# kv13arm/mujoco_rl_manipulate_unknown_objects

Hardware: NVIDIA B200
Metric: env-steps/sec (acorn_env, 4096 envs/GPU) (higher is better)
Workload: dtype f32

## Files before the change

mujoco_rl_manipulate_unknown_objects_b200/csrc/sim_kernels.cuh:

```cuda
#pragma once
#include <cuda_runtime.h>
#include <stdint.h>

#include "model.h"

namespace grs {

constexpr int MAXCON = 12;
constexpr int MAXEFC = MAXCON * 4 + 7;
constexpr unsigned FULL = 0xffffffffu;
constexpr float MINVAL = 1e-15f;

struct __align__(16) WS {
  float qpos[16], qvel[16], ctrl[8], warm[16];
  float xpos[MAXB][3], xquat[MAXB][4], xmat[MAXB][9];
  float xanchor[MAXJ][3], xaxis[MAXJ][3];
  float gpos[MAXG][3], gmat[MAXG][9];
  float com[MAXB][3];
  float cdof[16][6];
  float M[NV * NV];
  int ncon, nefc, nlim, overflow, coupled, padi[3];
  float c_dist[MAXCON], c_pos[MAXCON][3], c_frame[MAXCON][9], c_mu[MAXCON], c_fric[MAXCON][3];
  int c_g1[MAXCON], c_g2[MAXCON], c_pair[MAXCON];
  float fsmooth[16], asmooth[16], qacc[16], Ma[16], grad[16], search[16], Mv[16], fcon[16], bias[16];
  float e_D[MAXEFC], e_aref[MAXEFC], e_jar[MAXEFC], e_Jv[MAXEFC], e_force[MAXEFC], e_act[MAXEFC];
  float hc[MAXCON][16];
  int istate[32];
  float tgt[8], init_q[8], out[40];
  float sup[5][9];
  float cho[16];
  float sep[MAXPAIR][3];
  float gapb[MAXPAIR];
  float disp[MAXG];
  union {
    struct {
      float xipos[MAXB][3], ximat[MAXB][9], cinert[MAXB][10], crb[MAXB][10], cdofdot[16][6], cvel[MAXB][6], cfrc[MAXB][6];
      float L[NV * NV];
    } dyn;
    struct {
      float J[MAXEFC][NV];
      float H[NV * NV];
    } con;
  } u;
};

struct StepStats { int iters_total, max_iters, ncon_max; };

__device__ __forceinline__ float warp_sum(float v) {
#pragma unroll
  for (int o = 16; o > 0; o >>= 1) v += __shfl_xor_sync(FULL, v, o);
  return v;
}
__device__ __forceinline__ float dot3(const float* a, const float* b) { return a[0] * b[0] + a[1] * b[1] + a[2] * b[2]; }
__device__ __forceinline__ void cross3(float* r, const float* a, const float* b) {
  float x = a[1] * b[2] - a[2] * b[1], y = a[2] * b[0] - a[0] * b[2], z = a[0] * b[1] - a[1] * b[0];
  r[0] = x; r[1] = y; r[2] = z;
}
__device__ __forceinline__ float normalize3(float* a) {
  float n = sqrtf(dot3(a, a));
  if (n < MINVAL) { a[0] = 1; a[1] = 0; a[2] = 0; return n; }
  float inv = 1.0f / n;
  a[0] *= inv; a[1] *= inv; a[2] *= inv;
  return n;
}
__device__ __forceinline__ void quat_mul(float* r, const float* a, const float* b) {
  float t0 = a[0] * b[0] - a[1] * b[1] - a[2] * b[2] - a[3] * b[3];
  float t1 = a[0] * b[1] + a[1] * b[0] + a[2] * b[3] - a[3] * b[2];
  float t2 = a[0] * b[2] - a[1] * b[3] + a[2] * b[0] + a[3] * b[1];
  float t3 = a[0] * b[3] + a[1] * b[2] - a[2] * b[1] + a[3] * b[0];
  r[0] = t0; r[1] = t1; r[2] = t2; r[3] = t3;
}
__device__ __forceinline__ void quat_normalize(float* q) {
  float n = sqrtf(q[0] * q[0] + q[1] * q[1] + q[2] * q[2] + q[3] * q[3]);
  if (n < MINVAL) { q[0] = 1; q[1] = q[2] = q[3] = 0; return; }
  float inv = 1.0f / n;
  q[0] *= inv; q[1] *= inv; q[2] *= inv; q[3] *= inv;
}
__device__ __forceinline__ void quat2mat(float* R, const float* q) {
  float w = q[0], x = q[1], y = q[2], z = q[3];
  R[0] = w * w + x * x - y * y - z * z; R[1] = 2 * (x * y - w * z); R[2] = 2 * (x * z + w * y);
  R[3] = 2 * (x * y + w * z); R[4] = w * w - x * x + y * y - z * z; R[5] = 2 * (y * z - w * x);
  R[6] = 2 * (x * z - w * y); R[7] = 2 * (y * z + w * x); R[8] = w * w - x * x - y * y + z * z;
}
__device__ __forceinline__ void mulmat3vec(float* r, const float* R, const float* v) {
  float x = R[0] * v[0] + R[1] * v[1] + R[2] * v[2], y = R[3] * v[0] + R[4] * v[1] + R[5] * v[2], z = R[6] * v[0] + R[7] * v[1] + R[8] * v[2];
  r[0] = x; r[1] = y; r[2] = z;
}
__device__ __forceinline__ void mulmat3Tvec(float* r, const float* R, const float* v) {
  float x = R[0] * v[0] + R[3] * v[1] + R[6] * v[2], y = R[1] * v[0] + R[4] * v[1] + R[7] * v[2], z = R[2] * v[0] + R[5] * v[1] + R[8] * v[2];
  r[0] = x; r[1] = y; r[2] = z;
}
__device__ __forceinline__ void rot_vec_quat(float* r, const float* v, const float* q) {
  float R[9];
  quat2mat(R, q);
  mulmat3vec(r, R, v);
}
__device__ __forceinline__ void mul_inert_vec(float* r, const float* c, const float* v) {
  float t[3];
  r[0] = c[0] * v[0] + c[3] * v[1] + c[4] * v[2];
  r[1] = c[3] * v[0] + c[1] * v[1] + c[5] * v[2];
  r[2] = c[4] * v[0] + c[5] * v[1] + c[2] * v[2];
  cross3(t, c + 6, v + 3);
  r[0] += t[0]; r[1] += t[1]; r[2] += t[2];
  cross3(t, c + 6, v);
  r[3] = c[9] * v[3] - t[0]; r[4] = c[9] * v[4] - t[1]; r[5] = c[9] * v[5] - t[2];
}
__device__ __forceinline__ float dot6(const float* a, const float* b) { return a[0] * b[0] + a[1] * b[1] + a[2] * b[2] + a[3] * b[3] + a[4] * b[4] + a[5] * b[5]; }
__device__ __forceinline__ void cross_motion(float* r, const float* v, const float* mv) {
  float t[3];
  cross3(r, v, mv);
  cross3(r + 3, v, mv + 3);
  cross3(t, v + 3, mv);
  r[3] += t[0]; r[4] += t[1]; r[5] += t[2];
}
__device__ __forceinline__ void cross_force(float* r, const float* v, const float* f) {
  float t[3];
  cross3(r, v, f);
  cross3(t, v + 3, f + 3);
  r[0] += t[0]; r[1] += t[1]; r[2] += t[2];
  cross3(r + 3, v, f + 3);
}

template <bool BLOCKS>
__device__ __noinline__ float chol_factor_solve(float* A, float* tmp, float b, int lane) {
  constexpr int NB = BLOCKS ? 7 : NV;
  const bool is_row = lane < NV;
  const bool is_rhs = BLOCKS ? (lane == 13 || lane == 14) : (lane == NV);
  const int base = BLOCKS ? (((lane >= 7 && lane < NV) || lane == 14) ? 7 : 0) : 0;
  const int nb = BLOCKS ? (base ? 6 : 7) : NV;
  const int lr = is_rhs ? NB : lane - base;
  if (is_row) tmp[lane] = b;
  __syncwarp();
  float a[NB];
#pragma unroll
  for (int k = 0; k < NB; k++) {
    a[k] = 0.0f;
    if (k < nb) {
      if (is_row && k <= lr) a[k] = A[lane * NV + base + k];
      else if (is_rhs) a[k] = tmp[base + k];
    }
  }
#pragma unroll
  for (int j = 0; j < NB; j++) {
    if (is_row && lr >= j) A[lane * NV + base + j] = a[j];
    __syncwarp();
    const int cj = base + (j < nb ? j : 0);
    const float djj = A[cj * NV + cj];
    float rs = rsqrtf(fmaxf(djj, 1e-30f));
    rs = rs * (1.5f - 0.5f * djj * rs * rs);
    const float t = a[j] * rs * rs;
    a[j] *= rs;
#pragma unroll
    for (int k = j + 1; k < NB; k++) {
      const int rk = base + (k < nb ? k : 0);
      a[k] -= t * A[rk * NV + cj];
    }
  }
  __syncwarp();
  if (is_row) {
#pragma unroll
    for (int k = 0; k < NB; k++)
      if (k <= lr) A[lane * NV + base + k] = a[k];
  }
  if (is_rhs) {
#pragma unroll
    for (int k = 0; k < NB; k++)
      if (k < nb) tmp[base + k] = a[k];
  }
  __syncwarp();
  float y = is_row ? tmp[lane] : 0.0f;
#pragma unroll
  for (int j = NB - 1; j >= 0; j--) {
    const bool valid = j < nb;
    const int gj = base + (valid ? j : 0);
    const float ljj = A[gj * NV + gj];
    if (is_row && valid && lr == j) tmp[gj] = __fdividef(y, ljj);
    __syncwarp();
    const float xj = tmp[gj];
    if (is_row && valid) {
      if (lr == j) y = xj;
      else if (lr < j) y -= A[gj * NV + lane] * xj;
    }
  }
  __syncwarp();
  return y;
}

__device__ __noinline__ void kinematics(const DevModel& m, WS& w, int lane) {
  if (lane == 0) {
    for (int j = 0; j < m.njnt; j++)
      if (m.jnt_type[j] == JNT_FREE) quat_normalize(w.qpos + m.jnt_qposadr[j] + 3);
    w.xpos[0][0] = w.xpos[0][1] = w.xpos[0][2] = 0;
    w.xquat[0][0] = 1; w.xquat[0][1] = w.xquat[0][2] = w.xquat[0][3] = 0;
    quat2mat(w.xmat[0], w.xquat[0]);
  }
  __syncwarp();
  for (int lv = 1; lv < m.nlevel; lv++) {
    int idx = m.level_start[lv] + lane;
    if (idx < m.level_start[lv + 1]) {
      int b = m.level_body[idx], pid = m.body_parent[b];
      int jadr = m.body_jntadr[b], jnum = m.body_jntnum[b];
      float pos[3], quat[4];
      if (jnum == 1 && m.jnt_type[jadr] == JNT_FREE) {
        int qa = m.jnt_qposadr[jadr];
        for (int k = 0; k < 3; k++) pos[k] = w.qpos[qa + k];
        for (int k = 0; k < 4; k++) quat[k] = w.qpos[qa + 3 + k];
        for (int k = 0; k < 3; k++) { w.xanchor[jadr][k] = pos[k]; w.xaxis[jadr][k] = 0; }
      } else {
        float t[3];
        mulmat3vec(t, w.xmat[pid], m.body_pos[b]);
        for (int k = 0; k < 3; k++) pos[k] = w.xpos[pid][k] + t[k];
        quat_mul(quat, w.xquat[pid], m.body_quat[b]);
        for (int kj = 0; kj < jnum; kj++) {
          int j = jadr + kj;
          float anchor[3], axis[3];
          rot_vec_quat(t, m.jnt_pos[j], quat);
          for (int k = 0; k < 3; k++) anchor[k] = pos[k] + t[k];
          rot_vec_quat(axis, m.jnt_axis[j], quat);
          float q = w.qpos[m.jnt_qposadr[j]] - m.jnt_qpos0[j];
          if (m.jnt_type[j] == JNT_SLIDE) {
            for (int k = 0; k < 3; k++) pos[k] += axis[k] * q;
          } else {
            float s, c, ql[4];
            sincosf(0.5f * q, &s, &c);
            ql[0] = c; ql[1] = m.jnt_axis[j][0] * s; ql[2] = m.jnt_axis[j][1] * s; ql[3] = m.jnt_axis[j][2] * s;
            quat_mul(quat, quat, ql);
            rot_vec_quat(t, m.jnt_pos[j], quat);
            for (int k = 0; k < 3; k++) pos[k] = anchor[k] - t[k];
          }
          for (int k = 0; k < 3; k++) { w.xanchor[j][k] = anchor[k]; w.xaxis[j][k] = axis[k]; }
        }
      }
      quat_normalize(quat);
      for (int k = 0; k < 3; k++) w.xpos[b][k] = pos[k];
      for (int k = 0; k < 4; k++) w.xquat[b][k] = quat[k];
      quat2mat(w.xmat[b], quat);
    }
    __syncwarp();
  }
  if (lane < m.ngeom) {
    int g = lane, b = m.geom_body[g];
    float t[3], q[4], R[9];
    mulmat3vec(t, w.xmat[b], m.geom_pos[g]);
    quat_mul(q, w.xquat[b], m.geom_quat[g]);
    quat_normalize(q);
    quat2mat(R, q);
    float d2 = 0, r2 = 0;
    for (int k = 0; k < 3; k++) { const float np_ = w.xpos[b][k] + t[k], d = np_ - w.gpos[g][k]; d2 += d * d; w.gpos[g][k] = np_; }
    for (int k = 0; k < 9; k++) { const float d = R[k] - w.gmat[g][k]; r2 += d * d; w.gmat[g][k] = R[k]; }
    w.disp[g] = sqrtf(d2) + m.geom_rbound[g] * sqrtf(r2);
  }
  __syncwarp();
}

__device__ __noinline__ void com_pos_crb(const DevModel& m, WS& w, int lane) {
  const int nb = m.nbody;
  if (lane < nb) {
    int b = lane;
    float t[3], qi[4];
    mulmat3vec(t, w.xmat[b], m.body_ipos[b]);
    for (int k = 0; k < 3; k++) w.u.dyn.xipos[b][k] = w.xpos[b][k] + t[k];
    quat_mul(qi, w.xquat[b], m.body_iquat[b]);
    quat2mat(w.u.dyn.ximat[b], qi);
  }
  __syncwarp();
  if (lane < nb) {
    int r = m.body_root[lane];
    unsigned mask = m.body_subtree_mask[r];
    float s[3] = {0, 0, 0}, ms = 0;
    for (int b = 1; b < nb; b++)
      if ((mask >> b) & 1u) {
        float mb = m.body_mass[b];
        ms += mb;
        for (int k = 0; k < 3; k++) s[k] += mb * w.u.dyn.xipos[b][k];
      }
    if (ms < MINVAL) { for (int k = 0; k < 3; k++) w.com[lane][k] = w.u.dyn.xipos[r][k]; }
    else { float inv = 1.0f / ms; for (int k = 0; k < 3; k++) w.com[lane][k] = s[k] * inv; }
  }
  __syncwarp();
  if (lane < nb) {
    int b = lane;
    float* c = w.u.dyn.cinert[b];
    if (b == 0) { for (int k = 0; k < 10; k++) c[k] = 0; }
    else {
      const float* R = w.u.dyn.ximat[b];
      const float* I = m.body_inertia[b];
      float mb = m.body_mass[b], off[3];
      for (int k = 0; k < 3; k++) off[k] = w.u.dyn.xipos[b][k] - w.com[b][k];
      float dd = dot3(off, off);
      float M00 = R[0] * I[0] * R[0] + R[1] * I[1] * R[1] + R[2] * I[2] * R[2];
      float M11 = R[3] * I[0] * R[3] + R[4] * I[1] * R[4] + R[5] * I[2] * R[5];
      float M22 = R[6] * I[0] * R[6] + R[7] * I[1] * R[7] + R[8] * I[2] * R[8];
      float M01 = R[0] * I[0] * R[3] + R[1] * I[1] * R[4] + R[2] * I[2] * R[5];
      float M02 = R[0] * I[0] * R[6] + R[1] * I[1] * R[7] + R[2] * I[2] * R[8];
      float M12 = R[3] * I[0] * R[6] + R[4] * I[1] * R[7] + R[5] * I[2] * R[8];
      c[0] = M00 + mb * (dd - off[0] * off[0]);
      c[1] = M11 + mb * (dd - off[1] * off[1]);
      c[2] = M22 + mb * (dd - off[2] * off[2]);
      c[3] = M01 - mb * off[0] * off[1];
      c[4] = M02 - mb * off[0] * off[2];
      c[5] = M12 - mb * off[1] * off[2];
      c[6] = mb * off[0]; c[7] = mb * off[1]; c[8] = mb * off[2];
      c[9] = mb;
    }
  }
  if (lane < NV) {
    int i = lane, j = m.dof_jnt[i], b = m.dof_body[i], da = m.jnt_dofadr[j];
    float* c = w.cdof[i];
    int type = m.jnt_type[j];
    if (type == JNT_FREE) {
      int k = i - da;
      if (k < 3) { c[0] = c[1] = c[2] = 0; c[3] = k == 0; c[4] = k == 1; c[5] = k == 2; }
      else {
        k -= 3;
        float ax[3] = {w.xmat[b][k], w.xmat[b][3 + k], w.xmat[b][6 + k]}, off[3];
        for (int q = 0; q < 3; q++) off[q] = w.com[b][q] - w.xpos[b][q];
        c[0] = ax[0]; c[1] = ax[1]; c[2] = ax[2];
        cross3(c + 3, ax, off);
      }
    } else if (type == JNT_SLIDE) {
      c[0] = c[1] = c[2] = 0;
      for (int q = 0; q < 3; q++) c[3 + q] = w.xaxis[j][q];
    } else {
      float off[3], ax[3];
      for (int q = 0; q < 3; q++) { off[q] = w.com[b][q] - w.xanchor[j][q]; ax[q] = w.xaxis[j][q]; c[q] = ax[q]; }
      cross3(c + 3, ax, off);
    }
  }
  __syncwarp();
  if (lane < nb) {
    int b = lane;
    unsigned mask = m.body_subtree_mask[b];
    float acc[10];
    for (int k = 0; k < 10; k++) acc[k] = 0;
    if (b > 0)
      for (int bb = b; bb < nb; bb++)
        if ((mask >> bb) & 1u)
          for (int k = 0; k < 10; k++) acc[k] += w.u.dyn.cinert[bb][k];
// ... 274 lines not shown
        w.gapb[lane] = left;
        const bool has_axis = w.sep[lane][0] != 0.0f || w.sep[lane][1] != 0.0f || w.sep[lane][2] != 0.0f;
        if (cand && has_axis && left > 0.0f) cand = false;
      }
    }
  }
  unsigned todo = __ballot_sync(FULL, cand);
  __syncwarp();
  while (todo) {
    const int p = __ffs(todo) - 1;
    todo &= todo - 1;
    int g1 = m.pair_g1[p], g2 = m.pair_g2[p];
    float margin = m.pair_margin[p];
    if (m.geom_type[g1] == GEOM_PLANE) {
      const float* R1 = w.gmat[g1];
      float n[3] = {R1[2], R1[5], R1[8]}, dif[3];
      if (m.geom_type[g2] == GEOM_BOX) {
        for (int k = 0; k < 3; k++) dif[k] = w.gpos[g2][k] - w.gpos[g1][k];
        const float dist = dot3(dif, n);
        const int i = lane & 7;
        float vec[3] = {(i & 1) ? m.geom_size[g2][0] : -m.geom_size[g2][0], (i & 2) ? m.geom_size[g2][1] : -m.geom_size[g2][1],
                        (i & 4) ? m.geom_size[g2][2] : -m.geom_size[g2][2]}, corner[3];
        mulmat3vec(corner, w.gmat[g2], vec);
        const float ldist = dot3(n, corner);
        unsigned ok = __ballot_sync(FULL, lane < 8 && !(dist + ldist > margin || ldist > 0));
        for (int cnt = 0; ok && cnt < 4; cnt++) {
          const int src = __ffs(ok) - 1;
          ok &= ok - 1;
          float cd = __shfl_sync(FULL, dist + ldist, src), pos[3];
          for (int k = 0; k < 3; k++) pos[k] = __shfl_sync(FULL, corner[k], src) - 0.5f * cd * n[k] + w.gpos[g2][k];
          add_contact(m, w, p, cd, pos, n, lane);
        }
        continue;
      }
      float nn[3] = {-n[0], -n[1], -n[2]}, v[3], pos[3];
      int vi = support_geom(m, w, hv, g2, nn, v, lane);
      for (int k = 0; k < 3; k++) dif[k] = v[k] - w.gpos[g1][k];
      float dist = dot3(dif, n);
      if (dist > margin) continue;
      for (int k = 0; k < 3; k++) pos[k] = v[k] - 0.5f * dist * n[k];
      add_contact(m, w, p, dist, pos, n, lane);
      const int* ga = adj + m.geom_adjadr[g2];
      int nvert = m.geom_hvnum[g2];
      int e0 = __ldg(ga + vi), e1 = __ldg(ga + vi + 1), cnt = 1;
      const float4* hvg = hv + m.geom_hvadr[g2];
      for (int e = e0; e < e1 && cnt < 3; e++) {
        int nb = __ldg(ga + nvert + 1 + e);
        float4 q = hvg[nb];
        float qv[3] = {q.x, q.y, q.z}, t[3];
        mulmat3vec(t, w.gmat[g2], qv);
        for (int k = 0; k < 3; k++) { v[k] = w.gpos[g2][k] + t[k]; dif[k] = v[k] - w.gpos[g1][k]; }
        dist = dot3(dif, n);
        if (dist > margin) continue;
        for (int k = 0; k < 3; k++) pos[k] = v[k] - 0.5f * dist * n[k];
        add_contact(m, w, p, dist, pos, n, lane);
        cnt++;
      }
    } else {
      float depth, dir[3], pos[3];
      float ca[3] = {w.sep[p][0], w.sep[p][1], w.sep[p][2]};
      if (ca[0] != 0.0f || ca[1] != 0.0f || ca[2] != 0.0f) {
        support_md(m, w, hv, g1, g2, margin, ca, 4, lane);
        const float sd = dot3(SUPV(4), ca);
        if (sd < 0) {
          __syncwarp();
          if (lane == 0) w.gapb[p] = -sd - 2e-6f;
          __syncwarp();
          continue;
        }
      }
      bool hit = mpr_penetration(m, w, hv, g1, g2, margin, &depth, dir, pos, lane);
      __syncwarp();
      if (lane < 3) w.sep[p][lane] = hit ? 0.0f : dir[lane];
      if (lane == 3) w.gapb[p] = 0.0f;
      __syncwarp();
      if (!hit) continue;
      add_contact(m, w, p, margin - depth, pos, dir, lane);
    }
  }
  __syncwarp();
}

__device__ __forceinline__ void forward_position(const DevModel& m, WS& w, const float4* hv, const int* adj, int lane) {
  kinematics(m, w, lane);
  com_pos_crb(m, w, lane);
  collision(m, w, hv, adj, lane);
}

__device__ __noinline__ void smooth_forces(const DevModel& m, WS& w, int lane, bool actuation, float xfrc_z) {
  const int nb = m.nbody;
  if (lane == 0) for (int k = 0; k < 6; k++) { w.u.dyn.cvel[0][k] = 0; w.u.dyn.cfrc[0][k] = 0; }
  if (lane == 0) { float* a = w.u.dyn.crb[0]; a[0] = a[1] = a[2] = 0; a[3] = -m.gravity[0]; a[4] = -m.gravity[1]; a[5] = -m.gravity[2]; }
  __syncwarp();
  for (int lv = 1; lv < m.nlevel; lv++) {
    int idx = m.level_start[lv] + lane;
    if (idx < m.level_start[lv + 1]) {
      int b = m.level_body[idx], pid = m.body_parent[b];
      float cvel[6], cacc[6];
      for (int k = 0; k < 6; k++) { cvel[k] = w.u.dyn.cvel[pid][k]; cacc[k] = w.u.dyn.crb[pid][k]; }
      for (int kj = 0; kj < m.body_jntnum[b]; kj++) {
        int j = m.body_jntadr[b] + kj, a = m.jnt_dofadr[j];
        if (m.jnt_type[j] == JNT_FREE) {
          for (int i = 0; i < 3; i++) {
            for (int k = 0; k < 6; k++) w.u.dyn.cdofdot[a + i][k] = 0;
            float qv = w.qvel[a + i];
            for (int k = 0; k < 6; k++) cvel[k] += w.cdof[a + i][k] * qv;
          }
          float dd[3][6];
          for (int i = 0; i < 3; i++) cross_motion(dd[i], cvel, w.cdof[a + 3 + i]);
          for (int i = 0; i < 3; i++) {
            float qv = w.qvel[a + 3 + i];
            for (int k = 0; k < 6; k++) { w.u.dyn.cdofdot[a + 3 + i][k] = dd[i][k]; cvel[k] += w.cdof[a + 3 + i][k] * qv; cacc[k] += dd[i][k] * qv; }
          }
        } else {
          float dd[6], qv = w.qvel[a];
          cross_motion(dd, cvel, w.cdof[a]);
          for (int k = 0; k < 6; k++) { w.u.dyn.cdofdot[a][k] = dd[k]; cvel[k] += w.cdof[a][k] * qv; cacc[k] += dd[k] * qv; }
        }
      }
      float t1[6], t2[6], f[6];
      mul_inert_vec(t1, w.u.dyn.cinert[b], cacc);
      mul_inert_vec(t2, w.u.dyn.cinert[b], cvel);
      cross_force(f, cvel, t2);
      for (int k = 0; k < 6; k++) { w.u.dyn.cvel[b][k] = cvel[k]; w.u.dyn.crb[b][k] = cacc[k]; w.u.dyn.cfrc[b][k] = f[k] + t1[k]; }
    }
    __syncwarp();
  }
  float bias = 0;
  if (lane < NV) {
    int b = m.dof_body[lane];
    unsigned mask = m.body_subtree_mask[b];
    float acc[6] = {0, 0, 0, 0, 0, 0};
    for (int bb = b; bb < nb; bb++)
      if ((mask >> bb) & 1u)
        for (int k = 0; k < 6; k++) acc[k] += w.u.dyn.cfrc[bb][k];
    bias = dot6(w.cdof[lane], acc);
  }
  float f = 0;
  if (lane < NV) {
    f = -m.dof_damping[lane] * w.qvel[lane] - bias;
    if (actuation)
      for (int u = 0; u < NU; u++)
        if (m.act_dof[u] == lane) f += m.act_gear[u] * fminf(fmaxf(w.ctrl[u], m.act_lo[u]), m.act_hi[u]);
    if (xfrc_z != 0.0f && ((m.body_dofmask[m.body_ee] >> lane) & 1u)) {
      float off[3], t[3];
      for (int k = 0; k < 3; k++) off[k] = w.u.dyn.xipos[m.body_ee][k] - w.com[m.body_ee][k];
      cross3(t, w.cdof[lane], off);
      f += (w.cdof[lane][5] + t[2]) * xfrc_z;
    }
    w.bias[lane] = bias;
    w.fsmooth[lane] = f;
  }
  __syncwarp();
  for (int e = lane; e < NV * NV; e += 32) w.u.dyn.L[e] = w.M[e];
  __syncwarp();
  float a = chol_factor_solve<true>(w.u.dyn.L, w.cho, f, lane);
  if (lane < NV) w.asmooth[lane] = a;
  __syncwarp();
}

__device__ __noinline__ float get_impedance(const float* solimp, float pos, float margin) {
  if (solimp[0] == solimp[1] || solimp[2] <= MINVAL) return 0.5f * (solimp[0] + solimp[1]);
  float x = fabsf((pos - margin) / solimp[2]);
  if (x >= 1) return solimp[1];
  if (x <= 0) return solimp[0];
  float y, p = solimp[4], mid = solimp[3];
  if (p == 1.0f) y = x;
  else if (p == 2.0f) y = x <= mid ? x * x / mid : 1 - (1 - x) * (1 - x) / (1 - mid);
  else y = x <= mid ? powf(x, p) / powf(mid, p - 1) : 1 - powf(1 - x, p) / powf(1 - mid, p - 1);
  return solimp[0] + y * (solimp[1] - solimp[0]);
}

__device__ __noinline__ void make_constraint(const DevModel& m, WS& w, int lane) {
  bool active = false;
  float dist = 0, sign = 0;
  if (lane < m.njnt && m.jnt_limited[lane] && m.jnt_type[lane] != JNT_FREE) {
    float value = w.qpos[m.jnt_qposadr[lane]];
    float dl = value - m.jnt_range[lane][0], du = m.jnt_range[lane][1] - value;
    if (dl < 0) { active = true; dist = dl; sign = 1; }
    else if (du < 0) { active = true; dist = du; sign = -1; }
  }
  unsigned bal = __ballot_sync(FULL, active);
  int nlim = __popc(bal);
  int ncon = w.ncon;
  int nefc = nlim + 4 * ncon;
  for (int e = lane; e < nefc * NV; e += 32) (&w.u.con.J[0][0])[e] = 0;
  __syncwarp();
  const float h2 = 2 * m.timestep;
  if (active) {
    int r = __popc(bal & ((1u << lane) - 1));
    int dof = m.jnt_dofadr[lane];
    w.u.con.J[r][dof] = sign;
    float tc = fmaxf(m.jnt_solref[0], h2), dr = m.jnt_solref[1], dmax = m.jnt_solimp[1];
    float imp = get_impedance(m.jnt_solimp, dist, 0.0f);
    float R = fmaxf((1 - imp) * m.dof_invweight0[dof] / imp, MINVAL);
    float K = 1.0f / (dmax * dmax * tc * tc * dr * dr), B = 2.0f / (dmax * tc);
    w.e_D[r] = 1.0f / R;
    w.e_aref[r] = -B * sign * w.qvel[dof] - K * imp * dist;
  }
  if (lane < NV) {
    const int i = lane;
    for (int c = 0; c < ncon; c++) {
      int b1 = m.geom_body[w.c_g1[c]], b2 = m.geom_body[w.c_g2[c]];
      float jp[3] = {0, 0, 0}, jr[3] = {0, 0, 0};
      if ((m.body_dofmask[b2] >> i) & 1u) {
        float off[3], t[3];
        for (int k = 0; k < 3; k++) off[k] = w.c_pos[c][k] - w.com[b2][k];
        cross3(t, w.cdof[i], off);
        for (int k = 0; k < 3; k++) { jp[k] += w.cdof[i][3 + k] + t[k]; jr[k] += w.cdof[i][k]; }
      }
      if ((m.body_dofmask[b1] >> i) & 1u) {
        float off[3], t[3];
        for (int k = 0; k < 3; k++) off[k] = w.c_pos[c][k] - w.com[b1][k];
        cross3(t, w.cdof[i], off);
        for (int k = 0; k < 3; k++) { jp[k] -= w.cdof[i][3 + k] + t[k]; jr[k] -= w.cdof[i][k]; }
      }
      const float* f = w.c_frame[c];
      int r = nlim + 4 * c;
      w.u.con.J[r][i] = dot3(f, jp);
      w.u.con.J[r + 1][i] = dot3(f + 3, jp);
      w.u.con.J[r + 2][i] = dot3(f + 6, jp);
      w.u.con.J[r + 3][i] = dot3(f, jr);
    }
  }
  __syncwarp();
  if (lane < ncon) {
    int c = lane, p = w.c_pair[c], r = nlim + 4 * c;
    int b1 = m.geom_body[w.c_g1[c]], b2 = m.geom_body[w.c_g2[c]];
    float tran = m.body_invweight0[b1][0] + m.body_invweight0[b2][0];
    float tc = fmaxf(m.pair_solref[p][0], h2), dr = m.pair_solref[p][1], dmax = m.pair_solimp[p][1];
    float margin = m.pair_margin[p];
    float imp = get_impedance(m.pair_solimp[p], w.c_dist[c], margin);
    float R0 = fmaxf((1 - imp) * tran / imp, MINVAL);
    float R1 = R0 / fmaxf(MINVAL, m.impratio);
    float f0 = w.c_fric[c][0];
    float R2 = R1 * f0 * f0 / (w.c_fric[c][1] * w.c_fric[c][1]);
    float R3 = R1 * f0 * f0 / (w.c_fric[c][2] * w.c_fric[c][2]);
    w.c_mu[c] = f0 * sqrtf(R1 / R0);
    float K = 1.0f / (dmax * dmax * tc * tc * dr * dr), B = 2.0f / (dmax * tc);
    float vel[4];
    for (int j = 0; j < 4; j++) {
      float v = 0;
      for (int k = 0; k < NV; k++) v += w.u.con.J[r + j][k] * w.qvel[k];
      vel[j] = v;
    }
    w.e_D[r] = 1.0f / R0; w.e_D[r + 1] = 1.0f / R1; w.e_D[r + 2] = 1.0f / R2; w.e_D[r + 3] = 1.0f / R3;
    w.e_aref[r] = -B * vel[0] - K * imp * (w.c_dist[c] - margin);
    w.e_aref[r + 1] = -B * vel[1];
    w.e_aref[r + 2] = -B * vel[2];
    w.e_aref[r + 3] = -B * vel[3];
  }
  bool cpl = false;
  if (lane < ncon) {
    int r1 = m.body_root[m.geom_body[w.c_g1[lane]]], r2 = m.body_root[m.geom_body[w.c_g2[lane]]];
    cpl = r1 != 0 && r2 != 0 && r1 != r2;
  }
  cpl = __any_sync(FULL, cpl);
  if (lane == 0) { w.nefc = nefc; w.nlim = nlim; w.coupled = cpl; }
  __syncwarp();
}

__device__ __forceinline__ float constraint_update(WS& w, int lane, bool want_cone_hessian) {
  const int nlim = w.nlim, nitem = nlim + w.ncon;
  float cost = 0;
  int state = 0;
  if (lane < nlim) {
    float x = w.e_jar[lane];
    if (x < 0) { w.e_force[lane] = -w.e_D[lane] * x; cost = 0.5f * w.e_D[lane] * x * x; state = 1; w.e_act[lane] = w.e_D[lane]; }
    else { w.e_force[lane] = 0; w.e_act[lane] = 0; }
  } else if (lane < nitem) {
    int c = lane - nlim, r = nlim + 4 * c;
    float mu = w.c_mu[c], sc[4] = {mu, w.c_fric[c][0], w.c_fric[c][1], w.c_fric[c][2]};
    float U[4], T = 0;
    for (int j = 0; j < 4; j++) U[j] = w.e_jar[r + j] * sc[j];
    float N = U[0];
    T = sqrtf(U[1] * U[1] + U[2] * U[2] + U[3] * U[3]);
    if (N >= mu * T || (T <= 0 && N >= 0)) {
      for (int j = 0; j < 4; j++) { w.e_force[r + j] = 0; w.e_act[r + j] = 0; }
    } else if (mu * N + T <= 0 || (T <= 0 && N < 0)) {
      for (int j = 0; j < 4; j++) {
        float x = w.e_jar[r + j], D = w.e_D[r + j];
        w.e_force[r + j] = -D * x;
        cost += 0.5f * D * x * x;
        w.e_act[r + j] = D;
      }
      state = 1;
    } else {
      float Dm = w.e_D[r] / (mu * mu * (1 + mu * mu)), NmT = N - mu * T;
      cost = 0.5f * Dm * NmT * NmT;
      float f0 = -Dm * NmT * mu;
      w.e_force[r] = f0;
      for (int j = 1; j < 4; j++) w.e_force[r + j] = -f0 / T * U[j] * sc[j];
      for (int j = 0; j < 4; j++) w.e_act[r + j] = 0;
      state = 2;
      if (want_cone_hessian) {
        float* hc = w.hc[c];
        float invT = 1.0f / T;
        hc[0] = 1;
        for (int j = 1; j < 4; j++) { hc[j] = -mu * invT * U[j]; hc[4 * j] = hc[j]; }
        float scl = mu * N * invT * invT * invT;
        for (int j = 1; j < 4; j++)
          for (int k = 1; k < 4; k++) hc[4 * j + k] = scl * U[j] * U[k];
        float dg = mu * mu - mu * N * invT;
        for (int j = 1; j < 4; j++) hc[4 * j + j] += dg;
        for (int j = 0; j < 4; j++)
          for (int k = 0; k < 4; k++) hc[4 * j + k] *= Dm * sc[j] * sc[k];
      }
    }
  }
  w.istate[lane] = state;
  cost = warp_sum(cost);
  __syncwarp();
  return cost;
}

__device__ __forceinline__ void line_eval(const WS& w, int lane, float alpha, float q1, float q2, float& d1, float& d2) {
  const int nlim = w.nlim, nitem = nlim + w.ncon;
  float D1 = 0, D2 = 0;
  if (lane < nlim) {
    float x = w.e_jar[lane] + alpha * w.e_Jv[lane];
    if (x < 0) { float D = w.e_D[lane], jv = w.e_Jv[lane]; D1 = D * x * jv; D2 = D * jv * jv; }
  } else if (lane < nitem) {
    int c = lane - nlim, r = nlim + 4 * c;
    float mu = w.c_mu[c], sc[4] = {mu, w.c_fric[c][0], w.c_fric[c][1], w.c_fric[c][2]};
    float x[4], jv[4], U[4], V[4];
    for (int j = 0; j < 4; j++) { jv[j] = w.e_Jv[r + j]; x[j] = w.e_jar[r + j] + alpha * jv[j]; U[j] = x[j] * sc[j]; V[j] = jv[j] * sc[j]; }
    float TT = U[1] * U[1] + U[2] * U[2] + U[3] * U[3], T = sqrtf(TT), N = U[0];
    if (N >= mu * T || (T <= 0 && N >= 0)) {
    } else if (mu * N + T <= 0 || (T <= 0 && N < 0)) {
      for (int j = 0; j < 4; j++) { float D = w.e_D[r + j]; D1 += D * x[j] * jv[j]; D2 += D * jv[j] * jv[j]; }
    } else {
      float Dm = w.e_D[r] / (mu * mu * (1 + mu * mu)), NmT = N - mu * T;
      float UV = U[1] * V[1] + U[2] * V[2] + U[3] * V[3], VV = V[1] * V[1] + V[2] * V[2] + V[3] * V[3];
      float T1 = UV / T, T2 = (VV - T1 * T1) / T, a = V[0] - mu * T1;
      D1 = Dm * NmT * a;
      D2 = Dm * (a * a - NmT * mu * T2);
    }
  }
  D1 = warp_sum(D1);
  D2 = warp_sum(D2);
  d1 = q1 + alpha * q2 + D1;
  d2 = q2 + D2;
}

__device__ __forceinline__ float mat13_vec(const float* M, const float* x, int lane) {
  float v = 0;
  if (lane < NV) {
    const float* row = M + lane * NV;
#pragma unroll
    for (int k = 0; k < NV; k++) v += row[k] * x[k];
  }
  return v;
}
__device__ __forceinline__ void rows_dot(const WS& w, const float* x, const float* sub, float* out, int lane) {
#pragma unroll 1
  for (int r = lane; r < w.nefc; r += 32) {
    const float* row = w.u.con.J[r];
    float v = 0;
#pragma unroll
    for (int k = 0; k < NV; k++) v += row[k] * x[k];
    out[r] = sub ? v - sub[r] : v;
  }
}
__device__ __forceinline__ float jt_force(const WS& w, int lane) {
  float fc = 0;
  if (lane < NV) {
#pragma unroll 4
    for (int r = 0; r < w.nefc; r++) fc += w.u.con.J[r][lane] * w.e_force[r];
  }
  return fc;
}
__constant__ unsigned char HESS_TRI[91] = {
    0x00, 0x10, 0x11, 0x20, 0x21, 0x22, 0x30, 0x31, 0x32, 0x33, 0x40, 0x41, 0x42, 0x43, 0x44, 0x50, 0x51, 0x52, 0x53, 0x54, 0x55, 0x60, 0x61, 0x62, 0x63, 0x64,
    0x65, 0x66, 0x77, 0x87, 0x88, 0x97, 0x98, 0x99, 0xa7, 0xa8, 0xa9, 0xaa, 0xb7, 0xb8, 0xb9, 0xba, 0xbb, 0xc7, 0xc8, 0xc9, 0xca, 0xcb, 0xcc,
    0x70, 0x71, 0x72, 0x73, 0x74, 0x75, 0x76, 0x80, 0x81, 0x82, 0x83, 0x84, 0x85, 0x86, 0x90, 0x91, 0x92, 0x93, 0x94, 0x95, 0x96, 0xa0, 0xa1, 0xa2, 0xa3, 0xa4,
    0xa5, 0xa6, 0xb0, 0xb1, 0xb2, 0xb3, 0xb4, 0xb5, 0xb6, 0xc0, 0xc1, 0xc2, 0xc3, 0xc4, 0xc5, 0xc6};

__device__ __forceinline__ void make_hessian(WS& w, int lane) {
  const int nefc = w.nefc, nlim = w.nlim, ncon = w.ncon;
  const int nent = w.coupled ? 91 : 49;
#pragma unroll 1
  for (int i = lane; i < nent; i += 32) {
    const int ab = HESS_TRI[i], a = ab >> 4, b = ab & 15;
    float h = w.M[a * NV + b];
#pragma unroll 4
    for (int r = 0; r < nefc; r++) h += w.e_act[r] * w.u.con.J[r][a] * w.u.con.J[r][b];
#pragma unroll 1
    for (int c = 0; c < ncon; c++) {
      if (w.istate[nlim + c] != 2) continue;
      int r = nlim + 4 * c;
      const float* hc = w.hc[c];
      float jb0 = w.u.con.J[r][b], jb1 = w.u.con.J[r + 1][b], jb2 = w.u.con.J[r + 2][b], jb3 = w.u.con.J[r + 3][b];
#pragma unroll
      for (int j = 0; j < 4; j++) h += w.u.con.J[r + j][a] * (hc[4 * j] * jb0 + hc[4 * j + 1] * jb1 + hc[4 * j + 2] * jb2 + hc[4 * j + 3] * jb3);
    }
    w.u.con.H[a * NV + b] = h;
  }
  __syncwarp();
}

__device__ __noinline__ int solve_newton(const DevModel& m, WS& w, int lane, int max_iter) {
  const int nefc = w.nefc;
  float qa = 0;
  if (nefc == 0) {
    if (lane < NV) { w.qacc[lane] = w.asmooth[lane]; w.fcon[lane] = 0; }
    __syncwarp();
    return 0;
  }
  float best_cost = 0, gauss = 0;
#pragma unroll 1
  for (int trial = 0; trial < 2; trial++) {
    float q = lane < NV ? (trial == 0 ? w.warm[lane] : w.asmooth[lane]) : 0.0f;
    if (lane < NV) w.search[lane] = q;
    __syncwarp();
    float ma = mat13_vec(w.M, w.search, lane);
    rows_dot(w, w.search, w.e_aref, w.e_Jv, lane);
    float g = lane < NV ? 0.5f * (ma - w.fsmooth[lane]) * (q - w.asmooth[lane]) : 0.0f;
    g = warp_sum(g);
    __syncwarp();
    float keep0 = 0, keep1 = 0;
    if (lane < nefc) { keep0 = w.e_jar[lane]; w.e_jar[lane] = w.e_Jv[lane]; }
    if (lane + 32 < nefc) { keep1 = w.e_jar[lane + 32]; w.e_jar[lane + 32] = w.e_Jv[lane + 32]; }
    __syncwarp();
    float c = g + constraint_update(w, lane, false);
    if (trial == 0 || c < best_cost) {
      best_cost = c; gauss = g;
      if (lane < NV) { w.qacc[lane] = q; w.Ma[lane] = ma; }
      qa = q;
    } else {
      if (lane < nefc) w.e_jar[lane] = keep0;
      if (lane + 32 < nefc) w.e_jar[lane + 32] = keep1;
    }
    __syncwarp();
  }
  float cost = gauss + constraint_update(w, lane, true);
  const float scale = m.solver_scale;
  const float tol = 1e-8f;
  int iter = 0;
  float improvement = 0;
#pragma unroll 1
  for (; iter < max_iter; iter++) {
    float fc = jt_force(w, lane), g = 0;
    if (lane < NV) {
      g = w.Ma[lane] - w.fsmooth[lane] - fc;
      w.fcon[lane] = fc;
      w.grad[lane] = g;
    }
    float gn = scale * sqrtf(warp_sum(g * g));
    if (gn < tol) break;
    if (iter > 0 && improvement < tol) break;
    if (iter > 0 && m.newton_noise > 0.0f) {
      const float mag = lane < NV ? fabsf(w.Ma[lane]) + fabsf(w.fsmooth[lane]) + fabsf(fc) : 0.0f;
      if (gn < m.newton_noise * scale * sqrtf(warp_sum(mag * mag))) break;
    }
    __syncwarp();
    make_hessian(w, lane);
    float s = w.coupled ? chol_factor_solve<false>(w.u.con.H, w.cho, -g, lane) : chol_factor_solve<true>(w.u.con.H, w.cho, -g, lane);
    if (lane < NV) w.search[lane] = s;
    __syncwarp();
    float mv = mat13_vec(w.M, w.search, lane);
    if (lane < NV) w.Mv[lane] = mv;
    rows_dot(w, w.search, nullptr, w.e_Jv, lane);
    float q1 = lane < NV ? s * (w.Ma[lane] - w.fsmooth[lane]) : 0.0f;
    float q2 = lane < NV ? s * mv : 0.0f;
    float sn = lane < NV ? s * s : 0.0f;
    q1 = warp_sum(q1); q2 = warp_sum(q2); sn = sqrtf(warp_sum(sn));
    __syncwarp();
    if (sn < MINVAL) break;
    float d1, d2, alpha = 0, lo = 0, hi = -1;
    line_eval(w, lane, 0.0f, q1, q2, d1, d2);
    if (d1 >= 0 || d2 <= 0) break;
    const float gtol = 1e-6f * fabsf(d1);
    alpha = -d1 / d2;
#pragma unroll 1
    for (int it = 0; it < 20; it++) {
      line_eval(w, lane, alpha, q1, q2, d1, d2);
      if (fabsf(d1) < gtol) break;
      if (d1 < 0) lo = alpha; else hi = alpha;
      float an = alpha - d1 / d2;
      if (hi < 0) { if (an <= lo) an = 2 * lo + 1e-9f; }
      else if (!(an > lo && an < hi)) an = 0.5f * (lo + hi);
      if (hi > 0 && (hi - lo) < 1e-6f * hi) { alpha = 0.5f * (lo + hi); break; }
      alpha = an;
    }
    if (alpha <= 0) break;
    if (lane < NV) { qa += alpha * s; w.qacc[lane] = qa; w.Ma[lane] += alpha * mv; }
#pragma unroll 1
    for (int r = lane; r < nefc; r += 32) w.e_jar[r] += alpha * w.e_Jv[r];
    __syncwarp();
    float gs = lane < NV ? 0.5f * (w.Ma[lane] - w.fsmooth[lane]) * (qa - w.asmooth[lane]) : 0.0f;
    gs = warp_sum(gs);
    float old = cost;
    cost = gs + constraint_update(w, lane, true);
    improvement = scale * (old - cost);
  }
  if (iter == max_iter) {
    float fc = jt_force(w, lane);
    if (lane < NV) w.fcon[lane] = fc;
  }
  __syncwarp();
  return iter;
}

__device__ __noinline__ void euler_integrate(const DevModel& m, WS& w, int lane) {
  const float h = m.timestep;
#pragma unroll 1
  for (int e = lane; e < NV * NV; e += 32) {
    int a = e / NV, b = e - a * NV;
    w.u.con.H[e] = w.M[e] + (a == b ? h * m.dof_damping[a] : 0.0f);
  }
  __syncwarp();
  float f = lane < NV ? w.fsmooth[lane] + w.fcon[lane] : 0.0f;
  float qacc = chol_factor_solve<true>(w.u.con.H, w.cho, f, lane);
  if (lane < NV) {
    w.warm[lane] = w.qacc[lane];
    w.qvel[lane] += h * qacc;
  }
  __syncwarp();
  if (lane < m.njnt) {
    int j = lane, qa = m.jnt_qposadr[j], da = m.jnt_dofadr[j];
    if (m.jnt_type[j] == JNT_FREE) {
      for (int k = 0; k < 3; k++) w.qpos[qa + k] += h * w.qvel[da + k];
      float wv[3] = {w.qvel[da + 3], w.qvel[da + 4], w.qvel[da + 5]};
      float ang = sqrtf(dot3(wv, wv));
      if (ang > MINVAL) {
        float inv = 1.0f / ang, s, c, dq[4];
        sincosf(0.5f * ang * h, &s, &c);
        dq[0] = c; dq[1] = wv[0] * inv * s; dq[2] = wv[1] * inv * s; dq[3] = wv[2] * inv * s;
        float q[4] = {w.qpos[qa + 3], w.qpos[qa + 4], w.qpos[qa + 5], w.qpos[qa + 6]};
        quat_mul(q, q, dq);
        quat_normalize(q);
        for (int k = 0; k < 4; k++) w.qpos[qa + 3 + k] = q[k];
      }
    } else {
      w.qpos[qa] += h * w.qvel[da];
    }
  }
  __syncwarp();
}

__device__ __noinline__ int physics_step(const DevModel& m, WS& w, const float4* hv, const int* adj, int lane, float xfrc_z, bool actuation) {
  smooth_forces(m, w, lane, actuation, xfrc_z);
  make_constraint(m, w, lane);
  int it = solve_newton(m, w, lane, m.iterations);
  euler_integrate(m, w, lane);
  forward_position(m, w, hv, adj, lane);
  return it;
}

}
```

Measured before the change: 24.66 million.

## Factor mass matrix and damped integrator matrix together, reuse factor in Euler step

The smooth-dynamics Cholesky now factors both M and M+h*diag(damping) at once, using the two half-warps, and stores the damped factor plus the reciprocal pivots in new workspace arrays. The Euler integrator then only runs forward and back substitution on that stored factor instead of rebuilding and refactoring the matrix. Back substitution now broadcasts pivot values with warp shuffles instead of shared-memory round trips, and the Hessian build processes several entries per lane in registers. This adds workspace size and assumes M is unchanged between the dynamics and integration stages.

```diff
diff --git a/mujoco_rl_manipulate_unknown_objects_b200/csrc/sim_kernels.cuh b/mujoco_rl_manipulate_unknown_objects_b200/csrc/sim_kernels.cuh
--- a/mujoco_rl_manipulate_unknown_objects_b200/csrc/sim_kernels.cuh
+++ b/mujoco_rl_manipulate_unknown_objects_b200/csrc/sim_kernels.cuh
@@ -35,13 +35,14 @@
   union {
     struct {
       float xipos[MAXB][3], ximat[MAXB][9], cinert[MAXB][10], crb[MAXB][10], cdofdot[16][6], cvel[MAXB][6], cfrc[MAXB][6];
-      float L[NV * NV];
+      float L[NV * 7];
     } dyn;
     struct {
       float J[MAXEFC][NV];
       float H[NV * NV];
     } con;
   } u;
+  float Lh[NV * 7], rsh[NV];
 };
 
 struct StepStats { int iters_total, max_iters, ncon_max; };
@@ -121,6 +122,47 @@
   cross3(r + 3, v, f + 3);
 }
 
+
+template <int S>
+__device__ __forceinline__ int chol_at(int row, int base, int lcol) { return row * S + (S == NV ? base : 0) + lcol; }
+
+template <int NB, int S>
+__device__ __forceinline__ void chol_eliminate(float (&a)[NB], float* A, float* rs_out, int base, int nb, int lr, bool is_row) {
+#pragma unroll
+  for (int j = 0; j < NB; j++) {
+    const int jj = j < nb ? j : 0, cj = base + jj;
+    if (is_row && lr >= j) A[chol_at<S>(cj, base, lr)] = a[j];
+    __syncwarp();
+    const float djj = A[chol_at<S>(cj, base, jj)];
+    float rs = rsqrtf(fmaxf(djj, 1e-30f));
+    rs = rs * (1.5f - 0.5f * djj * rs * rs);
+    if (rs_out && is_row && lr == j) rs_out[base + lr] = rs;
+    const float t = a[j] * rs * rs;
+    a[j] *= rs;
+#pragma unroll
+    for (int k = j + 1; k < NB; k++) a[k] -= t * A[chol_at<S>(cj, base, k < nb ? k : 0)];
+  }
+}
+
+template <bool BLOCKS, int S>
+__device__ __forceinline__ float chol_back_subst(const float* A, float y, int lane) {
+  constexpr int NB = BLOCKS ? 7 : NV;
+  const int base = BLOCKS && lane >= 7 ? 7 : 0;
+  const int nb = BLOCKS ? (base ? 6 : 7) : NV;
+  const int lr = lane - base;
+#pragma unroll
+  for (int j = NB - 1; j >= 0; j--) {
+    const bool valid = j < nb;
+    const int jj = valid ? j : 0, gj = base + jj;
+    const float xj = __shfl_sync(FULL, __fdividef(y, A[chol_at<S>(gj, base, jj)]), gj);
+    if (lane < NV && valid) {
+      if (lr == j) y = xj;
+      else if (lr < j) y -= A[chol_at<S>(gj, base, lr)] * xj;
+    }
+  }
+  return y;
+}
+
 template <bool BLOCKS>
 __device__ __noinline__ float chol_factor_solve(float* A, float* tmp, float b, int lane) {
   constexpr int NB = BLOCKS ? 7 : NV;
@@ -140,22 +182,7 @@
       else if (is_rhs) a[k] = tmp[base + k];
     }
   }
-#pragma unroll
-  for (int j = 0; j < NB; j++) {
-    if (is_row && lr >= j) A[lane * NV + base + j] = a[j];
-    __syncwarp();
-    const int cj = base + (j < nb ? j : 0);
-    const float djj = A[cj * NV + cj];
-    float rs = rsqrtf(fmaxf(djj, 1e-30f));
-    rs = rs * (1.5f - 0.5f * djj * rs * rs);
-    const float t = a[j] * rs * rs;
-    a[j] *= rs;
-#pragma unroll
-    for (int k = j + 1; k < NB; k++) {
-      const int rk = base + (k < nb ? k : 0);
-      a[k] -= t * A[rk * NV + cj];
-    }
-  }
+  chol_eliminate<NB, NV>(a, A, nullptr, base, nb, lr, is_row);
   __syncwarp();
   if (is_row) {
 #pragma unroll
@@ -168,22 +195,71 @@
       if (k < nb) tmp[base + k] = a[k];
   }
   __syncwarp();
-  float y = is_row ? tmp[lane] : 0.0f;
-#pragma unroll
-  for (int j = NB - 1; j >= 0; j--) {
-    const bool valid = j < nb;
-    const int gj = base + (valid ? j : 0);
-    const float ljj = A[gj * NV + gj];
-    if (is_row && valid && lr == j) tmp[gj] = __fdividef(y, ljj);
-    __syncwarp();
-    const float xj = tmp[gj];
-    if (is_row && valid) {
-      if (lr == j) y = xj;
-      else if (lr < j) y -= A[gj * NV + lane] * xj;
-    }
-  }
-  __syncwarp();
-  return y;
+  return chol_back_subst<BLOCKS, NV>(A, is_row ? tmp[lane] : 0.0f, lane);
+}
+
+__device__ __noinline__ float chol_factor_pair(const float* M, float* L, float* Lh, float* rsh, float* tmp, float b, float hd, int lane) {
+  const int g = lane >> 4, row = lane & 15;
+  const bool is_row = row < NV, is_rhs = g == 0 && (row == 13 || row == 14);
+  const int base = ((row >= 7 && row < NV) || row == 14) ? 7 : 0;
+  const int nb = base ? 6 : 7, lr = is_rhs ? 7 : row - base;
+  float* A = g ? Lh : L;
+  if (lane < NV) tmp[lane] = b;
+  __syncwarp();
+  float a[7];
+#pragma unroll
+  for (int k = 0; k < 7; k++) {
+    a[k] = 0.0f;
+    if (k < nb) {
+      if (is_row && k <= lr) {
+        const float v = M[row * NV + base + k];
+        a[k] = g ? __fadd_rn(v, k == lr ? hd : 0.0f) : v;
+      } else if (is_rhs) {
+        a[k] = tmp[base + k];
+      }
+    }
+  }
+  chol_eliminate<7, 7>(a, A, g ? rsh : nullptr, base, nb, lr, is_row);
+  __syncwarp();
+  if (is_row) {
+#pragma unroll
+    for (int k = 0; k < 7; k++)
+      if (k <= lr) A[chol_at<7>(row, base, k)] = a[k];
+  }
+  if (is_rhs) {
+#pragma unroll
+    for (int k = 0; k < 7; k++)
+      if (k < nb) tmp[base + k] = a[k];
+  }
+  __syncwarp();
+  return chol_back_subst<true, 7>(L, lane < NV ? tmp[lane] : 0.0f, lane);
+}
+
+__device__ __noinline__ float chol_solve_pair(const float* A, const float* rs, float* tmp, float b, int lane) {
+  if (lane < NV) tmp[lane] = b;
+  __syncwarp();
+  if (lane == 13 || lane == 14) {
+    const int base = lane == 14 ? 7 : 0, nb = base ? 6 : 7;
+    float a[7];
+#pragma unroll
+    for (int k = 0; k < 7; k++) a[k] = k < nb ? tmp[base + k] : 0.0f;
+#pragma unroll
+    for (int j = 0; j < 7; j++) {
+      if (j >= nb) break;
+      const int cj = base + j;
+      const float r = rs[cj];
+      const float t = a[j] * r * r;
+      a[j] *= r;
+#pragma unroll
+      for (int k = j + 1; k < 7; k++)
+        if (k < nb) a[k] -= t * A[chol_at<7>(cj, base, k)];
+    }
+#pragma unroll
+    for (int k = 0; k < 7; k++)
+      if (k < nb) tmp[base + k] = a[k];
+  }
+  __syncwarp();
+  return chol_back_subst<true, 7>(A, lane < NV ? tmp[lane] : 0.0f, lane);
 }
 
 __device__ __noinline__ void kinematics(const DevModel& m, WS& w, int lane) {
@@ -764,9 +840,8 @@
     w.fsmooth[lane] = f;
   }
   __syncwarp();
-  for (int e = lane; e < NV * NV; e += 32) w.u.dyn.L[e] = w.M[e];
-  __syncwarp();
-  float a = chol_factor_solve<true>(w.u.dyn.L, w.cho, f, lane);
+  const float hd = lane >= 16 && lane < 16 + NV ? __fmul_rn(m.timestep, m.dof_damping[lane - 16]) : 0.0f;
+  float a = chol_factor_pair(w.M, w.u.dyn.L, w.Lh, w.rsh, w.cho, f, hd, lane);
   if (lane < NV) w.asmooth[lane] = a;
   __syncwarp();
 }
@@ -988,26 +1063,42 @@
     0x70, 0x71, 0x72, 0x73, 0x74, 0x75, 0x76, 0x80, 0x81, 0x82, 0x83, 0x84, 0x85, 0x86, 0x90, 0x91, 0x92, 0x93, 0x94, 0x95, 0x96, 0xa0, 0xa1, 0xa2, 0xa3, 0xa4,
     0xa5, 0xa6, 0xb0, 0xb1, 0xb2, 0xb3, 0xb4, 0xb5, 0xb6, 0xc0, 0xc1, 0xc2, 0xc3, 0xc4, 0xc5, 0xc6};
 
+template <int NQ>
+__device__ __forceinline__ void make_hessian_entries(WS& w, int lane, int nent) {
+  const int nefc = w.nefc, nlim = w.nlim, ncon = w.ncon;
+  int a[NQ], b[NQ];
+  float h[NQ];
+#pragma unroll
+  for (int q = 0; q < NQ; q++) {
+    const int i = lane + 32 * q, ab = HESS_TRI[i < nent ? i : 0];
+    a[q] = ab >> 4; b[q] = ab & 15;
+    h[q] = w.M[a[q] * NV + b[q]];
+  }
+#pragma unroll 4
+  for (int r = 0; r < nefc; r++) {
+    const float e = w.e_act[r];
+#pragma unroll
+    for (int q = 0; q < NQ; q++) h[q] += e * w.u.con.J[r][a[q]] * w.u.con.J[r][b[q]];
+  }
+#pragma unroll 1
+  for (int c = 0; c < ncon; c++) {
+    if (w.istate[nlim + c] != 2) continue;
+    int r = nlim + 4 * c;
+    const float* hc = w.hc[c];
+#pragma unroll
+    for (int q = 0; q < NQ; q++) {
+      float jb0 = w.u.con.J[r][b[q]], jb1 = w.u.con.J[r + 1][b[q]], jb2 = w.u.con.J[r + 2][b[q]], jb3 = w.u.con.J[r + 3][b[q]];
+#pragma unroll
+      for (int j = 0; j < 4; j++) h[q] += w.u.con.J[r + j][a[q]] * (hc[4 * j] * jb0 + hc[4 * j + 1] * jb1 + hc[4 * j + 2] * jb2 + hc[4 * j + 3] * jb3);
+    }
+  }
+#pragma unroll
+  for (int q = 0; q < NQ; q++)
+    if (lane + 32 * q < nent) w.u.con.H[a[q] * NV + b[q]] = h[q];
+}
 __device__ __forceinline__ void make_hessian(WS& w, int lane) {
-  const int nefc = w.nefc, nlim = w.nlim, ncon = w.ncon;
-  const int nent = w.coupled ? 91 : 49;
-#pragma unroll 1
-  for (int i = lane; i < nent; i += 32) {
-    const int ab = HESS_TRI[i], a = ab >> 4, b = ab & 15;
-    float h = w.M[a * NV + b];
-#pragma unroll 4
-    for (int r = 0; r < nefc; r++) h += w.e_act[r] * w.u.con.J[r][a] * w.u.con.J[r][b];
-#pragma unroll 1
-    for (int c = 0; c < ncon; c++) {
-      if (w.istate[nlim + c] != 2) continue;
-      int r = nlim + 4 * c;
-      const float* hc = w.hc[c];
-      float jb0 = w.u.con.J[r][b], jb1 = w.u.con.J[r + 1][b], jb2 = w.u.con.J[r + 2][b], jb3 = w.u.con.J[r + 3][b];
-#pragma unroll
-      for (int j = 0; j < 4; j++) h += w.u.con.J[r + j][a] * (hc[4 * j] * jb0 + hc[4 * j + 1] * jb1 + hc[4 * j + 2] * jb2 + hc[4 * j + 3] * jb3);
-    }
-    w.u.con.H[a * NV + b] = h;
-  }
+  if (w.coupled) make_hessian_entries<3>(w, lane, 91);
+  else make_hessian_entries<2>(w, lane, 49);
   __syncwarp();
 }
 
@@ -1116,14 +1207,8 @@
 
 __device__ __noinline__ void euler_integrate(const DevModel& m, WS& w, int lane) {
   const float h = m.timestep;
-#pragma unroll 1
-  for (int e = lane; e < NV * NV; e += 32) {
-    int a = e / NV, b = e - a * NV;
-    w.u.con.H[e] = w.M[e] + (a == b ? h * m.dof_damping[a] : 0.0f);
-  }
-  __syncwarp();
   float f = lane < NV ? w.fsmooth[lane] + w.fcon[lane] : 0.0f;
-  float qacc = chol_factor_solve<true>(w.u.con.H, w.cho, f, lane);
+  float qacc = chol_solve_pair(w.Lh, w.rsh, w.cho, f, lane);
   if (lane < NV) {
     w.warm[lane] = w.qacc[lane];
     w.qvel[lane] += h * qacc;
```

Result: slower. 24.12 million (median of 6 runs) (-2.2%).
